# ucas-vg/PointTinyBenchmark

Hardware: AMD Instinct MI355X
Metric: img/s (640x640) CPR R50-FPN fwd+loss (higher is better)
Workload: dtype fp32

## Files before the change

### pointtinybenchmark_amd/csrc/conv_wino.hip

```cpp
#include <type_traits>
#include "common.h"

typedef float f32x2 __attribute__((ext_vector_type(2)));
typedef int i32x4 __attribute__((ext_vector_type(4)));
typedef float f32x2 __attribute__((ext_vector_type(2)));

__device__ __forceinline__ f32x2 pk_add(f32x2 a, f32x2 b) {
    f32x2 r; asm("v_pk_add_f32 %0, %1, %2" : "=v"(r) : "v"(a), "v"(b)); return r;
}
__device__ __forceinline__ f32x2 pk_sub(f32x2 a, f32x2 b) {
    f32x2 r; asm("v_pk_add_f32 %0, %1, %2 neg_lo:[0,1] neg_hi:[0,1]" : "=v"(r) : "v"(a), "v"(b)); return r;
}
__device__ __forceinline__ f32x2 pk_col01(f32x2 t01, f32x2 t23) {
    f32x2 r; asm("v_pk_add_f32 %0, %1, %2 op_sel:[0,0] op_sel_hi:[1,0] neg_lo:[0,1] neg_hi:[0,0]" : "=v"(r) : "v"(t01), "v"(t23)); return r;
}
__device__ __forceinline__ f32x2 pk_col23(f32x2 t01, f32x2 t23) {
    f32x2 r; asm("v_pk_add_f32 %0, %1, %2 op_sel:[1,0] op_sel_hi:[1,1] neg_lo:[1,0] neg_hi:[0,1]" : "=v"(r) : "v"(t01), "v"(t23)); return r;
}
__device__ __forceinline__ f32x2 pk_fma(f32x2 a, f32x2 b, f32x2 c) {
    f32x2 r; asm("v_pk_fma_f32 %0, %1, %2, %3" : "=v"(r) : "v"(a), "v"(b), "v"(c)); return r;
}

struct WinoParams {
    const float* in;
    const float* u;
    float* out;
    const float* scale;
    const float* bias;
    float* gn_part;
    const float* in_a;
    const float* in_b;
    int in_relu, out_b8;
    int N, H, W, Cin, Cout, relu, RY, RX, regions, tilesN, nch;
    int tpx;
};

constexpr int WBUF = 16 * 64 * 8;

__global__ void wino_pack_kernel(const float* __restrict__ w, float* __restrict__ u, int Cin, int Cout, int Kpad) {
    const int idx = blockIdx.x * blockDim.x + threadIdx.x;
    if (idx >= Cin * Cout) return;
    const int ci = idx % Cin, co = idx / Cin;
    float g[3][3];
#pragma unroll
    for (int a = 0; a < 3; ++a)
#pragma unroll
        for (int b = 0; b < 3; ++b) g[a][b] = w[(size_t)co * Kpad + (a * 3 + b) * Cin + ci];
    float t[4][3];
#pragma unroll
    for (int b = 0; b < 3; ++b) {
        t[0][b] = g[0][b];
        t[1][b] = 0.5f * (g[0][b] + g[1][b] + g[2][b]);
        t[2][b] = 0.5f * (g[0][b] - g[1][b] + g[2][b]);
        t[3][b] = g[2][b];
    }
    const int tn = co >> 6, cl = co & 63, chunk = ci >> 3, k = ci & 7, nch = Cin >> 3;
    float* dst = u + ((size_t)(tn * nch + chunk) * 16) * 512 + cl * 8 + 4 * ((k >> 2) ^ ((cl >> 3) & 1)) + (k & 3);
#pragma unroll
    for (int i = 0; i < 4; ++i) {
        dst[(i * 4 + 0) * 512] = t[i][0];
        dst[(i * 4 + 1) * 512] = 0.5f * (t[i][0] + t[i][1] + t[i][2]);
        dst[(i * 4 + 2) * 512] = 0.5f * (t[i][0] - t[i][1] + t[i][2]);
        dst[(i * 4 + 3) * 512] = t[i][2];
    }
}

template <int ABL, bool INB8, bool XF, int TSPREAD = 1, int VAR = 0>
__global__ __launch_bounds__(512, 1) void conv_wino_kernel(WinoParams p) {
    constexpr bool DEEP = (VAR & 1) != 0, UDMA = (VAR & 4) != 0, USINGLE = (VAR & 2) != 0 && !UDMA;
    constexpr int XFMAX = 512;
    constexpr int RAWROW = 148;
    constexpr int RAWBUF = 18 * RAWROW;
    __shared__ __attribute__((aligned(16))) float smem[4 * WBUF + 2 * RAWBUF + (XF ? 4 * XFMAX : 0)];
    float* Vs = smem;
    float* Us = smem + 2 * WBUF;

    const int tid = threadIdx.x, lane = tid & 63;
    const int wave = __builtin_amdgcn_readfirstlane(tid >> 6);
    const int wi = wave & 3;
    const int nh = wave >> 2;

    const int pixbytes = INB8 ? 32 : p.Cin * 4;
    const int chunk_bytes = INB8 ? p.H * p.W * 32 : 32;
    const __amdgpu_buffer_rsrc_t rs_in = __builtin_amdgcn_make_buffer_rsrc(
        const_cast<float*>(p.in), 0, (int)((size_t)p.N * p.H * p.W * p.Cin * 4), 0x00020000);
    const __amdgpu_buffer_rsrc_t rs_u = __builtin_amdgcn_make_buffer_rsrc(
        const_cast<float*>(p.u), 0, (int)((size_t)p.tilesN * p.nch * WBUF * 4), 0x00020000);
    float* Rw = smem + 4 * WBUF;
    float* ABs = smem + 4 * WBUF + 2 * RAWBUF;
    int par = 0;
    int upyx[2], raw_wr[2];
#pragma unroll
    for (int k = 0; k < 2; ++k) {
        const int pix = (tid + 512 * k) >> 1;
        const int py = pix / 18, px = pix - py * 18;
        upyx[k] = py << 8 | px;
        raw_wr[k] = py * RAWROW + px * 8 + (tid & 1) * 4;
    }
    const bool second_unit = wave < 3;
    const bool unit1_live = tid + 512 < 648;
    const int lch = tid & 7, tyl = (tid >> 3) & 7, ltile = wave * 8 + tyl;
    const float* t_rd = Rw + (2 * tyl) * RAWROW + (2 * wave) * 8 + lch;
    const int v_wr = ltile * 8 + 4 * ((lch >> 2) ^ ((ltile >> 3) & 1)) + (lch & 3);
    const int last = p.nch - 1;
    const float relu_floor = (XF && p.in_relu) ? 0.f : -INFINITY;

    struct Tile {
        int rg, tn, n, oy0, ox0, n0;
        int voffA[2];
        unsigned uok;
        bool any_pad, valid;
    };
    const int T = p.regions * p.tilesN;
    const int per = (T + 7) >> 3;
    const int ngrp = p.tpx > 0 ? p.tilesN / p.tpx : 1;
    const int per_r = p.tpx > 0 ? (p.regions * ngrp + 7) / 8 : 0;
    auto setup = [&](int vb) {
        Tile t;
        if (p.tpx > 0) {
            const int x = vb & 7, s = vb >> 3;
            const int sr = s / p.tpx;
            t.rg = (x / ngrp) * per_r + sr;
            t.tn = (x % ngrp) * p.tpx + (s - sr * p.tpx);
            t.valid = sr < per_r && t.rg < p.regions;
            if (!t.valid) { t.rg = 0; t.tn = 0; }
        } else {
            const int tile = (vb & 7) * per + (vb >> 3);
            t.valid = vb < per * 8 && tile < T;
            const int tl = t.valid ? tile : 0;
            t.rg = tl / p.tilesN; t.tn = tl - t.rg * p.tilesN;
        }
        t.n = t.rg / (p.RY * p.RX);
        const int rrem = t.rg - t.n * p.RY * p.RX;
        const int ry = rrem / p.RX, rx = rrem - ry * p.RX;
        t.oy0 = ry * 16; t.ox0 = rx * 16; t.n0 = t.tn * 64;
        const int img_base = INB8 ? (t.n * (p.Cin >> 3)) * p.H * p.W * 32 : t.n * p.H * p.W * p.Cin * 4;
        t.uok = 0;
#pragma unroll
        for (int k = 0; k < 2; ++k) {
            const int iy = t.oy0 - 1 + (upyx[k] >> 8), ix = t.ox0 - 1 + (upyx[k] & 255);
            const bool ok = (k == 0 || unit1_live) & ((unsigned)iy < (unsigned)p.H) & ((unsigned)ix < (unsigned)p.W);
            t.uok |= (ok ? 1u : 0u) << k;
            t.voffA[k] = ok ? img_base + (iy * p.W + ix) * pixbytes + (tid & 1) * 16 : (int)0x80000000;
        }
        t.any_pad = XF && __builtin_amdgcn_ballot_w64(t.uok != (unit1_live ? 3u : 1u)) != 0;
        return t;
    };

    f32x4 sp[2][2];
    f32x4 su[(USINGLE || UDMA) ? 1 : 2][4];
    float tab_a = 0.f, tab_b = 0.f;
    f32x2 d[4][2];
    if (ABL & 9) { sp[0][0] = f32x4{1.f, 1.f, 1.f, 1.f}; sp[0][1] = sp[0][0]; sp[1][0] = sp[0][0]; sp[1][1] = sp[0][0]; }
    Tile cur = setup(blockIdx.x);
    auto ld_a = [&](const Tile& t, int ck, int k) {
        return __builtin_bit_cast(f32x4, __builtin_amdgcn_raw_buffer_load_b128(rs_in, t.voffA[k], ck * chunk_bytes, 0));
    };
    auto ld_u = [&](const Tile& t, int ck, int z) {
        return __builtin_bit_cast(
            f32x4, __builtin_amdgcn_raw_buffer_load_b128(rs_u, tid * 16 + z * 8192, (t.tn * p.nch + ck) * (WBUF * 4), 0));
    };
    auto prefetch = [&](const Tile& t) {
        if (!(ABL & 8)) {
            sp[0][0] = ld_a(t, 0, 0); sp[1][0] = ld_a(t, 1, 0);
            if (second_unit) { sp[0][1] = ld_a(t, 0, 1); sp[1][1] = ld_a(t, 1, 1); }
        }
        if (!UDMA) {
#pragma unroll
            for (int z = 0; z < 4; ++z) { su[0][z] = ld_u(t, 0, z); if (!USINGLE) su[USINGLE ? 0 : 1][z] = ld_u(t, 1, z); }
        }
        if (XF) {
            if (tid < p.Cin) { tab_a = p.in_a[t.n * p.Cin + tid]; tab_b = p.in_b[t.n * p.Cin + tid]; }
        }
    };
    auto g_a = [&](auto set_c, int chunk, int k) {
        constexpr int SET = decltype(set_c)::value;
        if (ABL & 8) return;
        const int ck = chunk < last ? chunk : last;
        if (k == 0 || second_unit) sp[SET][k] = ld_a(cur, ck, k);
    };
    auto g_u = [&](auto set_c, int chunk, int z) {
        constexpr int SET = (USINGLE || UDMA) ? 0 : decltype(set_c)::value;
        if (!UDMA) su[SET][z] = ld_u(cur, chunk < last ? chunk : last, z);
    };
    const int lds_u0 = (int)(unsigned)(size_t)(smem + 2 * WBUF);
    const size_t u_addr = (size_t)p.u;
    const i32x4 rs_u_raw = {(int)(unsigned)u_addr, (int)(unsigned)(u_addr >> 32) & 0xffff,
                            (int)((size_t)p.tilesN * p.nch * WBUF * 4), 0x00020000};
    auto dma_u = [&](int chunk, int buf, int z) {
        const int soff = (cur.tn * p.nch + chunk) * (WBUF * 4);
        const int m0v = lds_u0 + buf * (WBUF * 4) + z * 8192 + wave * 1024;
        asm volatile("s_nop 4\n\ts_mov_b32 m0, %0\n\ts_nop 0\n\tbuffer_load_dwordx4 %1, %2, %3 offen offset:0 lds"
                     :: "s"(m0v), "v"(tid * 16 + z * 8192), "s"(rs_u_raw), "s"(soff) : "memory");
    };
    auto dma_wait = [&](auto npatch_c) {
        constexpr int NP = decltype(npatch_c)::value;
        if (NP == 0) asm volatile("s_waitcnt vmcnt(0)" ::: "memory");
        else if (second_unit) asm volatile("s_waitcnt vmcnt(%0)" :: "n"(2 * NP) : "memory");
        else asm volatile("s_waitcnt vmcnt(%0)" :: "n"(NP) : "memory");
    };
    auto affine = [&](f32x4 v, f32x4 a4, f32x4 b4, int k) {
        if (ABL & 64) v = v * a4 + b4;
        else {
            const f32x2 lo = pk_fma(f32x2{v.x, v.y}, f32x2{a4.x, a4.y}, f32x2{b4.x, b4.y});
            const f32x2 hi = pk_fma(f32x2{v.z, v.w}, f32x2{a4.z, a4.w}, f32x2{b4.z, b4.w});
            v = f32x4{lo.x, lo.y, hi.x, hi.y};
        }
        v.x = fmaxf(v.x, relu_floor); v.y = fmaxf(v.y, relu_floor); v.z = fmaxf(v.z, relu_floor); v.w = fmaxf(v.w, relu_floor);
        if (cur.any_pad) {
            asm volatile("");
            if (!((cur.uok >> k) & 1u)) v = f32x4{0.f, 0.f, 0.f, 0.f};
        }
        return v;
    };
    f32x4 xa4, xb4;
    auto xf_fetch = [&](int chunk) {
        const float* tab = ABs + par * 2 * XFMAX + (chunk < last ? chunk : last) * 8 + (tid & 1) * 4;
        xa4 = *reinterpret_cast<const f32x4*>(tab);
        xb4 = *reinterpret_cast<const f32x4*>(tab + XFMAX);
    };
    auto r_a = [&](auto set_c, int buf, int k) {
        constexpr int SET = decltype(set_c)::value;
        if (k == 1 && !second_unit) return;
        f32x4 v = sp[SET][k];
        if (XF) v = affine(v, xa4, xb4, k);
        if (k == 0 || unit1_live) *reinterpret_cast<f32x4*>(Rw + buf * RAWBUF + raw_wr[k]) = v;
    };
    auto r_a_pro = [&](int chunk01, int k) {
        if (k == 1 && !second_unit) return;
        f32x4 v = chunk01 ? sp[1][k] : sp[0][k];
        if (XF) {
            const float* tab = ABs + par * 2 * XFMAX + chunk01 * 8 + (tid & 1) * 4;
            v = affine(v, *reinterpret_cast<const f32x4*>(tab), *reinterpret_cast<const f32x4*>(tab + XFMAX), k);
        }
        if (k == 0 || unit1_live) *reinterpret_cast<f32x4*>(Rw + chunk01 * RAWBUF + raw_wr[k]) = v;
    };
    auto r_u = [&](auto set_c, int buf, int z) {
        constexpr int SET = (USINGLE || UDMA) ? 0 : decltype(set_c)::value;
        if (!UDMA) *reinterpret_cast<f32x4*>(Us + buf * WBUF + tid * 4 + z * 2048) = su[SET][z];
    };
    auto t_read = [&](int buf, int r) {
#pragma unroll
        for (int s = 0; s < 2; ++s)
            d[r][s] = f32x2{t_rd[buf * RAWBUF + r * RAWROW + (2 * s) * 8], t_rd[buf * RAWBUF + r * RAWROW + (2 * s + 1) * 8]};
    };
    auto t_row = [&](int buf, int i) {
        float* dst = Vs + buf * WBUF + (i * 4) * 512 + v_wr;
        if (ABL & 64) {
            float ts[4];
#pragma unroll
            for (int s = 0; s < 4; ++s) {
                const float d0 = d[0][s >> 1][s & 1], d1 = d[1][s >> 1][s & 1], d2 = d[2][s >> 1][s & 1], d3 = d[3][s >> 1][s & 1];
                ts[s] = i == 0 ? d0 - d2 : i == 1 ? d1 + d2 : i == 2 ? d2 - d1 : d1 - d3;
            }
            dst[0 * 512] = ts[0] - ts[2];
            dst[1 * 512] = ts[1] + ts[2];
            dst[2 * 512] = ts[2] - ts[1];
            dst[3 * 512] = ts[1] - ts[3];
            return;
        }
        f32x2 t[2];
#pragma unroll
        for (int s = 0; s < 2; ++s)
            t[s] = i == 0 ? pk_sub(d[0][s], d[2][s]) : i == 1 ? pk_add(d[1][s], d[2][s]) : i == 2 ? pk_sub(d[2][s], d[1][s])
                                                                                                  : pk_sub(d[1][s], d[3][s]);
        const f32x2 o01 = pk_col01(t[0], t[1]), o23 = pk_col23(t[0], t[1]);
        dst[0 * 512] = o01.x;
        dst[1 * 512] = o01.y;
        dst[2 * 512] = o23.x;
        dst[3 * 512] = o23.y;
    };
    const int l31 = lane & 31, half = lane >> 5;
    const float* a_lds = Vs + (wi * 4 * 64 + l31) * 8 + 4 * (half ^ ((l31 >> 3) & 1));
    const float* b_lds = Us + (wi * 4 * 64 + nh * 32 + l31) * 8 + 4 * (half ^ ((l31 >> 3) & 1));
    using Set0 = std::integral_constant<int, 0>;
    using Set1 = std::integral_constant<int, 1>;

    if (cur.valid) prefetch(cur);
    if (XF) {
        if (tid < p.Cin) { ABs[tid] = tab_a; ABs[XFMAX + tid] = tab_b; }
        __syncthreads();
    }
    for (int vb = blockIdx.x; cur.valid; vb += gridDim.x) {
    const int rg = cur.rg, n = cur.n, oy0 = cur.oy0, ox0 = cur.ox0, n0 = cur.n0;

    f32x16 acc[4][2];
#pragma unroll
    for (int j = 0; j < 4; ++j)
#pragma unroll
        for (int tb = 0; tb < 2; ++tb)
#pragma unroll
            for (int r = 0; r < 16; ++r) acc[j][tb][r] = 0.f;

    f32x4 fa0[2], fb0, fa1[2], fb1;
#define WFRAG(FA, FB, buf, j, z)                                                                                    \
    do {                                                                                                            \
        if ((z) < 2) FA[(z) < 2 ? (z) : 0] = *reinterpret_cast<const f32x4*>(a_lds + (buf) * WBUF + (j) * 512 + ((z) < 2 ? (z) : 0) * 256); \
        else FB = *reinterpret_cast<const f32x4*>(b_lds + (buf) * WBUF + (j) * 512);                                \
    } while (0)
#define WMFMA(FA, FB, j, q) \
    acc[j][(q) & 1] = __builtin_amdgcn_mfma_f32_32x32x2f32(FA[(q) & 1][(q) >> 1], FB[(q) >> 1], acc[j][(q) & 1], 0, 0, 0)
    r_a_pro(0, 0); r_a_pro(0, 1);
    r_a_pro(1, 0); r_a_pro(1, 1);
    if (UDMA) {
#pragma unroll
        for (int z = 0; z < 4; ++z) dma_u(0, 0, z);
#pragma unroll
        for (int z = 0; z < 4; ++z) dma_u(1, 1, z);
    }
#pragma unroll
    for (int z = 0; z < 4; ++z) r_u(Set0{}, 0, z);
    g_a(Set0{}, 2, 0); g_a(Set0{}, 2, 1);
    if (DEEP) { g_a(Set1{}, 3, 0); g_a(Set1{}, 3, 1); }
#pragma unroll
    for (int z = 0; z < 4; ++z) g_u(Set0{}, USINGLE ? 1 : 2, z);
    __syncthreads();
#pragma unroll
    for (int r = 0; r < 4; ++r) t_read(0, r);
#pragma unroll
    for (int i = 0; i < 4; ++i) t_row(0, i);
    if (TSPREAD == 1) {
#pragma unroll
        for (int r = 0; r < 4; ++r) t_read(1, r);
    }
    if (UDMA) dma_wait(std::integral_constant<int, DEEP ? 2 : 1>{});
    __syncthreads();
#pragma unroll
    for (int z = 0; z < 3; ++z) WFRAG(fa0, fb0, 0, 0, z);

    auto iteration = [&](auto nxt_c, int c) {
        const int buf = c & 1;
        const std::integral_constant<int, DEEP ? 1 - decltype(nxt_c)::value : 0> pset_c{};
#pragma unroll
        for (int q = 0; q < 8; ++q) {
            WMFMA(fa0, fb0, 0, q);
            if (q < 3 && !(ABL & 2)) WFRAG(fa1, fb1, buf, 1, q);
            if (!(ABL & 1)) {
                if (TSPREAD == 0 || TSPREAD == 2) { if (q >= 4) t_read(buf ^ 1, q - 4); }
                else { if (q == 3) t_row(buf ^ 1, 0); if (q == 6) t_row(buf ^ 1, 1); }
            }
            __builtin_amdgcn_sched_barrier(0);
        }
#pragma unroll
        for (int q = 0; q < 8; ++q) {
            WMFMA(fa1, fb1, 1, q);
            if (q < 3 && !(ABL & 2)) WFRAG(fa0, fb0, buf, 2, q);
            if (!(ABL & 1)) {
                if (q & 1) r_u(nxt_c, buf ^ 1, q >> 1);
                else if (TSPREAD == 0) t_row(buf ^ 1, q >> 1);
                else if (TSPREAD == 2) {
                    if (q == 0) {
#pragma unroll
                        for (int i = 0; i < 4; ++i) t_row(buf ^ 1, i);
                    }
                }
                else if (q == 2) t_row(buf ^ 1, 2);
                else if (q == 6) t_row(buf ^ 1, 3);
                if (XF && q == 7) xf_fetch(c + 2);
            }
            __builtin_amdgcn_sched_barrier(0);
        }
#pragma unroll
        for (int q = 0; q < 8; ++q) {
            WMFMA(fa0, fb0, 2, q);
            if (q < 3 && !(ABL & 2)) WFRAG(fa1, fb1, buf, 3, q);
            if (!(ABL & 1)) {
                if (q == 3) { r_a(pset_c, buf, 0); if (TSPREAD == 2) r_a(pset_c, buf, 1); }
                if (q == 4 && TSPREAD != 2) r_a(pset_c, buf, 1);
                if (q == 5 || q == 6 || q == 7) g_u(nxt_c, c + (USINGLE ? 2 : 3), q - 5);
            }
            __builtin_amdgcn_sched_barrier(0);
        }
        asm volatile("" ::: "memory");
        if (UDMA) dma_wait(std::integral_constant<int, DEEP ? 1 : 0>{});
        __builtin_amdgcn_s_waitcnt(0xc07f);
        if (!(ABL & 4)) __builtin_amdgcn_s_barrier();
        asm volatile("" ::: "memory");
        __builtin_amdgcn_sched_barrier(0);
#pragma unroll
        for (int q = 0; q < 8; ++q) {
            WMFMA(fa1, fb1, 3, q);
            if (q < 3 && !(ABL & 2)) WFRAG(fa0, fb0, buf ^ 1, 0, q);
            if (!(ABL & 1)) {
                if (UDMA) {
                    if (q < 4 && c + 2 < p.nch) dma_u(c + 2, buf, q);
                    if (q == 4) g_a(pset_c, c + (DEEP ? 4 : 3), 0);
                    if (q == 6) g_a(pset_c, c + (DEEP ? 4 : 3), 1);
                } else {
                    if (q == 3) g_a(pset_c, c + (DEEP ? 4 : 3), 0);
                    if (q == 5) g_a(pset_c, c + (DEEP ? 4 : 3), 1);
                    if (q == 7) g_u(nxt_c, c + (USINGLE ? 2 : 3), 3);
                }
                if (TSPREAD == 1 && q >= 4) t_read(buf, q - 4);
            }
            __builtin_amdgcn_sched_barrier(0);
        }
    };
    for (int c = 0; c < p.nch; c += 2) {
        iteration(Set1{}, c);
        iteration(Set0{}, c + 1);
    }
#undef WFRAG
#undef WMFMA

    if (ABL & 32) {
        asm volatile("" ::"v"(acc[0][0]), "v"(acc[0][1]), "v"(acc[1][0]), "v"(acc[1][1]));
        asm volatile("" ::"v"(acc[2][0]), "v"(acc[2][1]), "v"(acc[3][0]), "v"(acc[3][1]));
        cur = setup(vb + gridDim.x);
        if (cur.valid) prefetch(cur);
        if (XF && tid < p.Cin) { ABs[(par ^ 1) * 2 * XFMAX + tid] = tab_a; ABs[(par ^ 1) * 2 * XFMAX + XFMAX + tid] = tab_b; }
        par ^= 1;
        __syncthreads();
        continue;
    }
    const Tile nxt = setup(vb + gridDim.x);
    if (nxt.valid) prefetch(nxt);
    __syncthreads();
    float* Rs = smem;
#pragma unroll
    for (int tb = 0; tb < 2; ++tb)
#pragma unroll
        for (int r = 0; r < 16; ++r) {
            const int trow = tb * 32 + (r & 3) + 8 * (r >> 2) + 4 * half;
            const float m0 = acc[0][tb][r], m1 = acc[1][tb][r], m2 = acc[2][tb][r], m3 = acc[3][tb][r];
            Rs[((wi * 2 + 0) * 64 + trow) * 64 + nh * 32 + l31] = m0 + m1 + m2;
            Rs[((wi * 2 + 1) * 64 + trow) * 64 + nh * 32 + l31] = m1 - m2 - m3;
        }
    __syncthreads();
    const int c4 = tid & 15;
    const int co = n0 + c4 * 4;
    f32x4 sc = {1.f, 1.f, 1.f, 1.f}, bi = {0.f, 0.f, 0.f, 0.f};
    if (p.scale) sc = *reinterpret_cast<const f32x4*>(p.scale + co);
    if (p.bias) bi = *reinterpret_cast<const f32x4*>(p.bias + co);
    const __amdgpu_buffer_rsrc_t rs_out = __builtin_amdgcn_make_buffer_rsrc(
        p.out, 0, (int)((size_t)p.N * p.H * p.W * p.Cout * 4), 0x00020000);
    f32x4 gs = {0.f, 0.f, 0.f, 0.f}, gq = {0.f, 0.f, 0.f, 0.f};
#pragma unroll
    for (int k = 0; k < 2; ++k) {
        const int t = (tid >> 4) + 32 * k;
        const int oy = oy0 + 2 * (t & 7), ox = ox0 + 2 * (t >> 3);
#pragma unroll
        for (int b = 0; b < 2; ++b) {
            const f32x4 r0 = *reinterpret_cast<const f32x4*>(Rs + ((0 * 2 + b) * 64 + t) * 64 + c4 * 4);
            const f32x4 r1 = *reinterpret_cast<const f32x4*>(Rs + ((1 * 2 + b) * 64 + t) * 64 + c4 * 4);
            const f32x4 r2 = *reinterpret_cast<const f32x4*>(Rs + ((2 * 2 + b) * 64 + t) * 64 + c4 * 4);
            const f32x4 r3 = *reinterpret_cast<const f32x4*>(Rs + ((3 * 2 + b) * 64 + t) * 64 + c4 * 4);
            f32x4 y[2] = {r0 + r1 + r2, r1 - r2 - r3};
#pragma unroll
            for (int a = 0; a < 2; ++a) {
                f32x4 v = y[a] * sc + bi;
                if (p.relu) { v.x = fmaxf(v.x, 0.f); v.y = fmaxf(v.y, 0.f); v.z = fmaxf(v.z, 0.f); v.w = fmaxf(v.w, 0.f); }
                const bool ok = (oy + a < p.H) & (ox + b < p.W);
                const unsigned off = !ok ? 0x80000000u
                    : p.out_b8 ? (unsigned)((((n * (p.Cout >> 3) + (co >> 3)) * p.H + oy + a) * p.W + ox + b) * 8 + (co & 7)) * 4u
                               : (unsigned)(((n * p.H + oy + a) * p.W + ox + b) * p.Cout + co) * 4u;
                if (!(ABL & 16)) __builtin_amdgcn_raw_buffer_store_b128(__builtin_bit_cast(__attribute__((ext_vector_type(4))) unsigned, v), rs_out, (int)off, 0, 0);
                if (p.gn_part && ok) { gs += v; gq += v * v; }
            }
        }
    }
    if (p.gn_part) {
#pragma unroll
        for (int e = 0; e < 4; ++e) {
            gs[e] += __shfl_xor(gs[e], 16, 64); gs[e] += __shfl_xor(gs[e], 32, 64);
            gq[e] += __shfl_xor(gq[e], 16, 64); gq[e] += __shfl_xor(gq[e], 32, 64);
        }
        __syncthreads();
        if (lane < 16) {
#pragma unroll
            for (int e = 0; e < 4; ++e) {
                smem[(wave * 64 + c4 * 4 + e) * 2 + 0] = gs[e];
                smem[(wave * 64 + c4 * 4 + e) * 2 + 1] = gq[e];
            }
        }
        __syncthreads();
        if (tid < 64) {
            float s = 0.f, q = 0.f;
#pragma unroll
            for (int w8 = 0; w8 < 8; ++w8) { s += smem[(w8 * 64 + tid) * 2]; q += smem[(w8 * 64 + tid) * 2 + 1]; }
            float* dst = p.gn_part + ((size_t)rg * p.Cout + n0 + tid) * 2;
            dst[0] = s; dst[1] = q;
        }
    }
    if (XF && tid < p.Cin) {
        ABs[(par ^ 1) * 2 * XFMAX + tid] = tab_a;
        ABs[(par ^ 1) * 2 * XFMAX + XFMAX + tid] = tab_b;
    }
    par ^= 1;
    __syncthreads();
    cur = nxt;
    }
}

#ifdef CPR_BENCH_HOOKS
static int wino_sched = 0, wino_ablate = 0, wino_var = -1, wino_tpx = -1;
extern "C" int cpr_wino_set_variant(int sched, int ablate) {
    CPR_CHECK_ARG(sched >= 0 && sched <= 2 && ablate >= 0 && ablate <= 64);
    wino_sched = sched;
    wino_ablate = ablate;
    return CPR_OK;
}
extern "C" int cpr_wino_set_staging(int var, int tpx) {
    CPR_CHECK_ARG(var >= -1 && var <= 5 && tpx >= -1 && tpx <= 2);
    wino_var = var;
    wino_tpx = tpx;
    return CPR_OK;
}
#else
constexpr int wino_sched = 0, wino_ablate = 0, wino_var = -1, wino_tpx = -1;
#endif
constexpr int WINO_VAR_DEFAULT = 4, WINO_TPX_DEFAULT = 0;
extern "C" int cpr_wino_pack_weights(const float* wgt, float* u, int Cin, int Cout, int Kpad, hipStream_t stream) {
    CPR_CHECK_ARG(wgt && u && Cin > 0 && Cout > 0 && Cin % 8 == 0 && Cout % 64 == 0 && Kpad >= 9 * Cin);
    hipLaunchKernelGGL(wino_pack_kernel, dim3(cdiv(Cin * Cout, 256)), dim3(256), 0, stream, wgt, u, Cin, Cout, Kpad);
    CPR_LAUNCH_STATUS();
}
static int wino_fwd_launch(const float* in, const float* u, float* out, const float* scale, const float* bias,
                           const float* in_a, const float* in_b, float* gn_part, int N, int H, int W, int Cin,
                           int Cout, int flags, int in_relu, int layout, hipStream_t stream) {
    CPR_CHECK_ARG(in && u && out && N > 0 && H > 0 && W > 0);
    CPR_CHECK_ARG(Cin > 0 && Cout > 0 && Cin % 16 == 0 && Cout % 64 == 0 && Cin >= 32);
    CPR_CHECK_ARG((flags & ~CPR_CONV_RELU) == 0 && (layout & ~3) == 0);
    if (in_a) CPR_CHECK_ARG(in_b && Cin <= 512);
    if ((long long)N * H * W * Cin * 4 >= (1ll << 31) || (long long)N * H * W * Cout * 4 >= (1ll << 31)) return CPR_ERR_UNSUPPORTED;
    WinoParams p;
    p.in = in; p.u = u; p.out = out; p.scale = scale; p.bias = bias; p.gn_part = gn_part;
    p.in_a = in_a; p.in_b = in_b; p.in_relu = in_relu; p.out_b8 = (layout & CPR_WINO_OUT_B8) ? 1 : 0;
    p.N = N; p.H = H; p.W = W; p.Cin = Cin; p.Cout = Cout; p.relu = flags & CPR_CONV_RELU;
    p.RY = (H + 15) / 16; p.RX = (W + 15) / 16;
    p.regions = N * p.RY * p.RX; p.tilesN = Cout / 64; p.nch = Cin / 8;
    const long long T = (long long)p.regions * p.tilesN;
    if (T >= (1ll << 30)) return CPR_ERR_UNSUPPORTED;
    static int cu_of_device[64] = {};
    int dev = 0, ncu = 256;
    if (hipGetDevice(&dev) == hipSuccess && dev >= 0 && dev < 64) {
        if (cu_of_device[dev] == 0) {
            int v = 0;
            if (hipDeviceGetAttribute(&v, hipDeviceAttributeMultiprocessorCount, dev) == hipSuccess && v > 0) cu_of_device[dev] = v;
        }
        if (cu_of_device[dev] > 0) ncu = cu_of_device[dev];
    }
    ncu = (ncu + 7) / 8 * 8;
    int grid = (int)((T + 7) / 8 * 8);
    if (grid > ncu) grid = ncu;
    const bool b8 = (layout & CPR_WINO_IN_B8) != 0, xf = in_a != nullptr;
    p.tpx = wino_tpx >= 0 ? wino_tpx : WINO_TPX_DEFAULT;
    if (p.tpx > 0 && !(p.tilesN % p.tpx == 0 && 8 % (p.tilesN / p.tpx) == 0)) p.tpx = 0;
    if (p.tpx > 0) {
        const long long per_r = ((long long)p.regions * (p.tilesN / p.tpx) + 7) / 8;
        const long long vbs = 8 * per_r * p.tpx;
        if (vbs < grid) grid = (int)vbs;
    }
    const int var = wino_var >= 0 ? wino_var : WINO_VAR_DEFAULT;
#define WLAUNCHV(A_, F_, V_)                                                                                                      \
    do {                                                                                                                         \
        constexpr int TX_ = F_ == 2 ? 2 : 0 ^ F_, TP_ = F_ == 2 ? 2 : 1 ^ F_;                                                     \
        if (b8 && xf) hipLaunchKernelGGL((conv_wino_kernel<A_, true, true, TX_, V_>), dim3(grid), dim3(512), 0, stream, p);       \
        else if (b8) hipLaunchKernelGGL((conv_wino_kernel<A_, true, false, TP_, V_>), dim3(grid), dim3(512), 0, stream, p);       \
        else if (xf) hipLaunchKernelGGL((conv_wino_kernel<A_, false, true, TX_, V_>), dim3(grid), dim3(512), 0, stream, p);       \
        else hipLaunchKernelGGL((conv_wino_kernel<A_, false, false, TP_, V_>), dim3(grid), dim3(512), 0, stream, p);              \
    } while (0)
#define WLAUNCH(A_, F_) WLAUNCHV(A_, F_, WINO_VAR_DEFAULT)
#ifdef CPR_BENCH_HOOKS
    if ((var != WINO_VAR_DEFAULT || wino_sched == 2) && !wino_ablate) {
        switch (var * 3 + wino_sched) {
            case 0: WLAUNCHV(0, 0, 0); break;
            case 1: WLAUNCHV(0, 1, 0); break;
            case 2: WLAUNCHV(0, 2, 0); break;
            case 6: WLAUNCHV(0, 0, 2); break;
            case 7: WLAUNCHV(0, 1, 2); break;
            case 8: WLAUNCHV(0, 2, 2); break;
            case 9: WLAUNCHV(0, 0, 3); break;
            case 10: WLAUNCHV(0, 1, 3); break;
            case 11: WLAUNCHV(0, 2, 3); break;
            case 12: WLAUNCHV(0, 0, 4); break;
            case 13: WLAUNCHV(0, 1, 4); break;
            case 14: WLAUNCHV(0, 2, 4); break;
            default: return CPR_ERR_UNSUPPORTED;
        }
    } else if (wino_ablate || wino_sched) {
        switch (wino_ablate) {
            case 0: WLAUNCH(0, 1); break;
            case 1: WLAUNCH(1, 0); break;
            case 2: WLAUNCH(2, 0); break;
            case 4: WLAUNCH(4, 0); break;
            case 8: WLAUNCH(8, 0); break;
            case 16: WLAUNCH(16, 0); break;
            case 32: WLAUNCH(32, 0); break;
            case 64: WLAUNCH(64, 0); break;
            default: WLAUNCH(7, 0); break;
        }
    } else
#endif
    WLAUNCH(0, 0);
#undef WLAUNCH
#undef WLAUNCHV
    CPR_LAUNCH_STATUS();
}

extern "C" int cpr_conv3x3_wino_fwd(const float* in, const float* u, float* out, const float* scale, const float* bias,
                                    const float* in_a, const float* in_b, float* gn_part, int N, int H, int W, int Cin,
                                    int Cout, int flags, int in_relu, int layout, hipStream_t stream) {
    CPR_CHECK_ARG(N > 0 && H > 0 && W > 0 && Cin > 0 && Cout > 0);
    const int per = cpr_images_per_launch(N, (long long)H * W * cpr_max2(Cin, Cout) * 4);
    if (per <= 0) return CPR_ERR_UNSUPPORTED;
    const size_t slots = (size_t)((H + 15) / 16) * ((W + 15) / 16);
    for (int n0 = 0; n0 < N; n0 += per) {
        const int n = N - n0 < per ? N - n0 : per;
        const int rc = wino_fwd_launch(in + (size_t)n0 * H * W * Cin, u, out + (size_t)n0 * H * W * Cout, scale, bias,
                                       in_a ? in_a + (size_t)n0 * Cin : nullptr, in_b ? in_b + (size_t)n0 * Cin : nullptr,
                                       gn_part ? gn_part + (size_t)n0 * slots * Cout * 2 : nullptr, n, H, W, Cin, Cout, flags,
                                       in_relu, layout, stream);
        if (rc != CPR_OK) return rc;
    }
    return CPR_OK;
}
```

Baseline: 898.7.

## Overlap Winograd output epilogue with next tile's prologue staging

```diff
diff --git a/pointtinybenchmark_amd/csrc/conv_wino.hip b/pointtinybenchmark_amd/csrc/conv_wino.hip
--- a/pointtinybenchmark_amd/csrc/conv_wino.hip
+++ b/pointtinybenchmark_amd/csrc/conv_wino.hip
@@ -68,6 +68,7 @@
 template <int ABL, bool INB8, bool XF, int TSPREAD = 1, int VAR = 0>
 __global__ __launch_bounds__(512, 1) void conv_wino_kernel(WinoParams p) {
     constexpr bool DEEP = (VAR & 1) != 0, UDMA = (VAR & 4) != 0, USINGLE = (VAR & 2) != 0 && !UDMA;
+    constexpr bool OVERLAP = XF;
     constexpr int XFMAX = 512;
     constexpr int RAWROW = 148;
     constexpr int RAWBUF = 18 * RAWROW;
@@ -160,16 +161,18 @@
         return __builtin_bit_cast(
             f32x4, __builtin_amdgcn_raw_buffer_load_b128(rs_u, tid * 16 + z * 8192, (t.tn * p.nch + ck) * (WBUF * 4), 0));
     };
-    auto prefetch = [&](const Tile& t) {
+    auto prefetch = [&](const Tile& t, bool table) {
         if (!(ABL & 8)) {
-            sp[0][0] = ld_a(t, 0, 0); sp[1][0] = ld_a(t, 1, 0);
-            if (second_unit) { sp[0][1] = ld_a(t, 0, 1); sp[1][1] = ld_a(t, 1, 1); }
+            sp[0][0] = ld_a(t, 0, 0);
+            if (second_unit) sp[0][1] = ld_a(t, 0, 1);
+            sp[1][0] = ld_a(t, 1, 0);
+            if (second_unit) sp[1][1] = ld_a(t, 1, 1);
         }
         if (!UDMA) {
 #pragma unroll
             for (int z = 0; z < 4; ++z) { su[0][z] = ld_u(t, 0, z); if (!USINGLE) su[USINGLE ? 0 : 1][z] = ld_u(t, 1, z); }
         }
-        if (XF) {
+        if (XF && table) {
             if (tid < p.Cin) { tab_a = p.in_a[t.n * p.Cin + tid]; tab_b = p.in_b[t.n * p.Cin + tid]; }
         }
     };
@@ -199,6 +202,12 @@
         else if (second_unit) asm volatile("s_waitcnt vmcnt(%0)" :: "n"(2 * NP) : "memory");
         else asm volatile("s_waitcnt vmcnt(%0)" :: "n"(NP) : "memory");
     };
+    auto dma_wait_boundary = [&](auto npatch_c) {
+        constexpr int NP = (ABL & 8) ? 0 : decltype(npatch_c)::value;
+        constexpr int OLD = ((ABL & 16) ? 0 : 8) + 4;
+        if (second_unit) asm volatile("s_waitcnt vmcnt(%0)" :: "n"(OLD + 2 * NP) : "memory");
+        else asm volatile("s_waitcnt vmcnt(%0)" :: "n"(OLD + NP) : "memory");
+    };
     auto affine = [&](f32x4 v, f32x4 a4, f32x4 b4, int k) {
         if (ABL & 64) v = v * a4 + b4;
         else {
@@ -276,13 +285,48 @@
     using Set0 = std::integral_constant<int, 0>;
     using Set1 = std::integral_constant<int, 1>;
 
-    if (cur.valid) prefetch(cur);
+    auto head_plain = [&]() {
+        r_a_pro(0, 0); r_a_pro(0, 1);
+        r_a_pro(1, 0); r_a_pro(1, 1);
+        if (UDMA) {
+#pragma unroll
+            for (int z = 0; z < 4; ++z) dma_u(0, 0, z);
+#pragma unroll
+            for (int z = 0; z < 4; ++z) dma_u(1, 1, z);
+        }
+#pragma unroll
+        for (int z = 0; z < 4; ++z) r_u(Set0{}, 0, z);
+        g_a(Set0{}, 2, 0); g_a(Set0{}, 2, 1);
+        if (DEEP) { g_a(Set1{}, 3, 0); g_a(Set1{}, 3, 1); }
+#pragma unroll
+        for (int z = 0; z < 4; ++z) g_u(Set0{}, USINGLE ? 1 : 2, z);
+        __syncthreads();
+#pragma unroll
+        for (int r = 0; r < 4; ++r) t_read(0, r);
+#pragma unroll
+        for (int i = 0; i < 4; ++i) t_row(0, i);
+        if (TSPREAD == 1) {
+#pragma unroll
+            for (int r = 0; r < 4; ++r) t_read(1, r);
+        }
+        if (UDMA) dma_wait(std::integral_constant<int, (ABL & 8) ? 0 : DEEP ? 2 : 1>{});
+        __syncthreads();
+    };
+
+    if (cur.valid) prefetch(cur, true);
     if (XF) {
         if (tid < p.Cin) { ABs[tid] = tab_a; ABs[XFMAX + tid] = tab_b; }
         __syncthreads();
     }
+    if (cur.valid) head_plain();
     for (int vb = blockIdx.x; cur.valid; vb += gridDim.x) {
     const int rg = cur.rg, n = cur.n, oy0 = cur.oy0, ox0 = cur.ox0, n0 = cur.n0;
+
+    const int c4 = tid & 15;
+    const int co = n0 + c4 * 4;
+    f32x4 sc = {1.f, 1.f, 1.f, 1.f}, bi = {0.f, 0.f, 0.f, 0.f};
+    if (p.scale) sc = *reinterpret_cast<const f32x4*>(p.scale + co);
+    if (p.bias) bi = *reinterpret_cast<const f32x4*>(p.bias + co);
 
     f32x16 acc[4][2];
 #pragma unroll
@@ -300,31 +344,6 @@
     } while (0)
 #define WMFMA(FA, FB, j, q) \
     acc[j][(q) & 1] = __builtin_amdgcn_mfma_f32_32x32x2f32(FA[(q) & 1][(q) >> 1], FB[(q) >> 1], acc[j][(q) & 1], 0, 0, 0)
-    r_a_pro(0, 0); r_a_pro(0, 1);
-    r_a_pro(1, 0); r_a_pro(1, 1);
-    if (UDMA) {
-#pragma unroll
-        for (int z = 0; z < 4; ++z) dma_u(0, 0, z);
-#pragma unroll
-        for (int z = 0; z < 4; ++z) dma_u(1, 1, z);
-    }
-#pragma unroll
-    for (int z = 0; z < 4; ++z) r_u(Set0{}, 0, z);
-    g_a(Set0{}, 2, 0); g_a(Set0{}, 2, 1);
-    if (DEEP) { g_a(Set1{}, 3, 0); g_a(Set1{}, 3, 1); }
-#pragma unroll
-    for (int z = 0; z < 4; ++z) g_u(Set0{}, USINGLE ? 1 : 2, z);
-    __syncthreads();
-#pragma unroll
-    for (int r = 0; r < 4; ++r) t_read(0, r);
-#pragma unroll
-    for (int i = 0; i < 4; ++i) t_row(0, i);
-    if (TSPREAD == 1) {
-#pragma unroll
-        for (int r = 0; r < 4; ++r) t_read(1, r);
-    }
-    if (UDMA) dma_wait(std::integral_constant<int, DEEP ? 2 : 1>{});
-    __syncthreads();
 #pragma unroll
     for (int z = 0; z < 3; ++z) WFRAG(fa0, fb0, 0, 0, z);
 
@@ -396,10 +415,12 @@
             __builtin_amdgcn_sched_barrier(0);
         }
     };
-    for (int c = 0; c < p.nch; c += 2) {
+    int c = 0;
+    do {
         iteration(Set1{}, c);
         iteration(Set0{}, c + 1);
-    }
+        c += 2;
+    } while (c < p.nch);
 #undef WFRAG
 #undef WMFMA
 
@@ -407,44 +428,114 @@
         asm volatile("" ::"v"(acc[0][0]), "v"(acc[0][1]), "v"(acc[1][0]), "v"(acc[1][1]));
         asm volatile("" ::"v"(acc[2][0]), "v"(acc[2][1]), "v"(acc[3][0]), "v"(acc[3][1]));
         cur = setup(vb + gridDim.x);
-        if (cur.valid) prefetch(cur);
+        if (cur.valid) prefetch(cur, true);
         if (XF && tid < p.Cin) { ABs[(par ^ 1) * 2 * XFMAX + tid] = tab_a; ABs[(par ^ 1) * 2 * XFMAX + XFMAX + tid] = tab_b; }
         par ^= 1;
         __syncthreads();
+        if (cur.valid) head_plain();
         continue;
     }
-    const Tile nxt = setup(vb + gridDim.x);
-    if (nxt.valid) prefetch(nxt);
-    __syncthreads();
-    float* Rs = smem;
-#pragma unroll
-    for (int tb = 0; tb < 2; ++tb)
-#pragma unroll
-        for (int r = 0; r < 16; ++r) {
-            const int trow = tb * 32 + (r & 3) + 8 * (r >> 2) + 4 * half;
-            const float m0 = acc[0][tb][r], m1 = acc[1][tb][r], m2 = acc[2][tb][r], m3 = acc[3][tb][r];
-            Rs[((wi * 2 + 0) * 64 + trow) * 64 + nh * 32 + l31] = m0 + m1 + m2;
-            Rs[((wi * 2 + 1) * 64 + trow) * 64 + nh * 32 + l31] = m1 - m2 - m3;
-        }
-    __syncthreads();
-    const int c4 = tid & 15;
-    const int co = n0 + c4 * 4;
-    f32x4 sc = {1.f, 1.f, 1.f, 1.f}, bi = {0.f, 0.f, 0.f, 0.f};
-    if (p.scale) sc = *reinterpret_cast<const f32x4*>(p.scale + co);
-    if (p.bias) bi = *reinterpret_cast<const f32x4*>(p.bias + co);
     const __amdgpu_buffer_rsrc_t rs_out = __builtin_amdgcn_make_buffer_rsrc(
         p.out, 0, (int)((size_t)p.N * p.H * p.W * p.Cout * 4), 0x00020000);
-    f32x4 gs = {0.f, 0.f, 0.f, 0.f}, gq = {0.f, 0.f, 0.f, 0.f};
-#pragma unroll
-    for (int k = 0; k < 2; ++k) {
-        const int t = (tid >> 4) + 32 * k;
-        const int oy = oy0 + 2 * (t & 7), ox = ox0 + 2 * (t >> 3);
-#pragma unroll
-        for (int b = 0; b < 2; ++b) {
-            const f32x4 r0 = *reinterpret_cast<const f32x4*>(Rs + ((0 * 2 + b) * 64 + t) * 64 + c4 * 4);
-            const f32x4 r1 = *reinterpret_cast<const f32x4*>(Rs + ((1 * 2 + b) * 64 + t) * 64 + c4 * 4);
-            const f32x4 r2 = *reinterpret_cast<const f32x4*>(Rs + ((2 * 2 + b) * 64 + t) * 64 + c4 * 4);
-            const f32x4 r3 = *reinterpret_cast<const f32x4*>(Rs + ((3 * 2 + b) * 64 + t) * 64 + c4 * 4);
+    if (!OVERLAP) {
+        cur = setup(vb + gridDim.x);
+        if (cur.valid) prefetch(cur, true);
+        __syncthreads();
+        float* Rs = smem;
+#pragma unroll
+        for (int tb = 0; tb < 2; ++tb)
+#pragma unroll
+            for (int r = 0; r < 16; ++r) {
+                const int trow = tb * 32 + (r & 3) + 8 * (r >> 2) + 4 * half;
+                const float m0 = acc[0][tb][r], m1 = acc[1][tb][r], m2 = acc[2][tb][r], m3 = acc[3][tb][r];
+                Rs[((wi * 2 + 0) * 64 + trow) * 64 + nh * 32 + l31] = m0 + m1 + m2;
+                Rs[((wi * 2 + 1) * 64 + trow) * 64 + nh * 32 + l31] = m1 - m2 - m3;
+            }
+        __syncthreads();
+        f32x4 gs = {0.f, 0.f, 0.f, 0.f}, gq = {0.f, 0.f, 0.f, 0.f};
+#pragma unroll
+        for (int k = 0; k < 2; ++k) {
+            const int t = (tid >> 4) + 32 * k;
+            const int oy = oy0 + 2 * (t & 7), ox = ox0 + 2 * (t >> 3);
+#pragma unroll
+            for (int b = 0; b < 2; ++b) {
+                const f32x4 r0 = *reinterpret_cast<const f32x4*>(Rs + ((0 * 2 + b) * 64 + t) * 64 + c4 * 4);
+                const f32x4 r1 = *reinterpret_cast<const f32x4*>(Rs + ((1 * 2 + b) * 64 + t) * 64 + c4 * 4);
+                const f32x4 r2 = *reinterpret_cast<const f32x4*>(Rs + ((2 * 2 + b) * 64 + t) * 64 + c4 * 4);
+                const f32x4 r3 = *reinterpret_cast<const f32x4*>(Rs + ((3 * 2 + b) * 64 + t) * 64 + c4 * 4);
+                f32x4 y[2] = {r0 + r1 + r2, r1 - r2 - r3};
+#pragma unroll
+                for (int a = 0; a < 2; ++a) {
+                    f32x4 v = y[a] * sc + bi;
+                    if (p.relu) { v.x = fmaxf(v.x, 0.f); v.y = fmaxf(v.y, 0.f); v.z = fmaxf(v.z, 0.f); v.w = fmaxf(v.w, 0.f); }
+                    const bool ok = (oy + a < p.H) & (ox + b < p.W);
+                    const unsigned off = !ok ? 0x80000000u
+                        : p.out_b8 ? (unsigned)((((n * (p.Cout >> 3) + (co >> 3)) * p.H + oy + a) * p.W + ox + b) * 8 + (co & 7)) * 4u
+                                   : (unsigned)(((n * p.H + oy + a) * p.W + ox + b) * p.Cout + co) * 4u;
+                    if (!(ABL & 16)) __builtin_amdgcn_raw_buffer_store_b128(__builtin_bit_cast(__attribute__((ext_vector_type(4))) unsigned, v), rs_out, (int)off, 0, 0);
+                    if (p.gn_part && ok) { gs += v; gq += v * v; }
+                }
+            }
+        }
+        if (p.gn_part) {
+#pragma unroll
+            for (int e = 0; e < 4; ++e) {
+                gs[e] += __shfl_xor(gs[e], 16, 64); gs[e] += __shfl_xor(gs[e], 32, 64);
+                gq[e] += __shfl_xor(gq[e], 16, 64); gq[e] += __shfl_xor(gq[e], 32, 64);
+            }
+            __syncthreads();
+            if (lane < 16) {
+#pragma unroll
+                for (int e = 0; e < 4; ++e) {
+                    smem[(wave * 64 + c4 * 4 + e) * 2 + 0] = gs[e];
+                    smem[(wave * 64 + c4 * 4 + e) * 2 + 1] = gq[e];
+                }
+            }
+            __syncthreads();
+            if (tid < 64) {
+                float s = 0.f, q = 0.f;
+#pragma unroll
+                for (int w8 = 0; w8 < 8; ++w8) { s += smem[(w8 * 64 + tid) * 2]; q += smem[(w8 * 64 + tid) * 2 + 1]; }
+                float* dst = p.gn_part + ((size_t)rg * p.Cout + n0 + tid) * 2;
+                dst[0] = s; dst[1] = q;
+            }
+        }
+        __syncthreads();
+        if (cur.valid) head_plain();
+        continue;
+    }
+    cur = setup(vb + gridDim.x);
+    const bool stage = cur.valid;
+    const bool new_table = XF && stage && cur.n != n;
+    if (stage) {
+        if (UDMA) {
+#pragma unroll
+            for (int z = 0; z < 4; ++z) dma_u(0, 0, z);
+        }
+        prefetch(cur, new_table);
+    }
+    float* r_wr = smem + WBUF + (wi >> 1) * 2 * WBUF + (wi & 1) * 4096 + nh * 32 + l31;
+    auto r_pass = [&](int b) {
+#pragma unroll
+        for (int tb = 0; tb < 2; ++tb)
+#pragma unroll
+            for (int r = 0; r < 16; ++r) {
+                const int trow = tb * 32 + (r & 3) + 8 * (r >> 2) + 4 * half;
+                const float m0 = acc[0][tb][r], m1 = acc[1][tb][r], m2 = acc[2][tb][r], m3 = acc[3][tb][r];
+                r_wr[trow * 64] = b == 0 ? m0 + m1 + m2 : m1 - m2 - m3;
+            }
+    };
+    f32x4 yv[2][2][2];
+    auto y_pass = [&](int b) {
+#pragma unroll
+        for (int k = 0; k < 2; ++k) {
+            const int t = (tid >> 4) + 32 * k;
+            const int oy = oy0 + 2 * (t & 7), ox = ox0 + 2 * (t >> 3);
+            const float* r_rd = smem + WBUF + t * 64 + c4 * 4;
+            const f32x4 r0 = *reinterpret_cast<const f32x4*>(r_rd);
+            const f32x4 r1 = *reinterpret_cast<const f32x4*>(r_rd + 4096);
+            const f32x4 r2 = *reinterpret_cast<const f32x4*>(r_rd + 2 * WBUF);
+            const f32x4 r3 = *reinterpret_cast<const f32x4*>(r_rd + 2 * WBUF + 4096);
             f32x4 y[2] = {r0 + r1 + r2, r1 - r2 - r3};
 #pragma unroll
             for (int a = 0; a < 2; ++a) {
@@ -455,40 +546,87 @@
                     : p.out_b8 ? (unsigned)((((n * (p.Cout >> 3) + (co >> 3)) * p.H + oy + a) * p.W + ox + b) * 8 + (co & 7)) * 4u
                                : (unsigned)(((n * p.H + oy + a) * p.W + ox + b) * p.Cout + co) * 4u;
                 if (!(ABL & 16)) __builtin_amdgcn_raw_buffer_store_b128(__builtin_bit_cast(__attribute__((ext_vector_type(4))) unsigned, v), rs_out, (int)off, 0, 0);
-                if (p.gn_part && ok) { gs += v; gq += v * v; }
-            }
-        }
-    }
+                yv[b][k][a] = v;
+            }
+        }
+    };
+
+    r_pass(0);
+    if (new_table) {
+        if (tid < p.Cin) { ABs[(par ^ 1) * 2 * XFMAX + tid] = tab_a; ABs[(par ^ 1) * 2 * XFMAX + XFMAX + tid] = tab_b; }
+        par ^= 1;
+    }
+    __syncthreads();
+    y_pass(0);
+    __syncthreads();
+    r_pass(1);
+    if (stage) {
+        r_a_pro(0, 0); r_a_pro(0, 1);
+        r_a_pro(1, 0); r_a_pro(1, 1);
+#pragma unroll
+        for (int z = 0; z < 4; ++z) r_u(Set0{}, 0, z);
+    }
+    __syncthreads();
+    if (stage) {
+#pragma unroll
+        for (int r = 0; r < 4; ++r) t_read(0, r);
+#pragma unroll
+        for (int i = 0; i < 4; ++i) t_row(0, i);
+    }
+    y_pass(1);
+    float* Gs = ABs + (par ^ 1) * 2 * XFMAX;
     if (p.gn_part) {
+        f32x4 gs = {0.f, 0.f, 0.f, 0.f}, gq = {0.f, 0.f, 0.f, 0.f};
+#pragma unroll
+        for (int k = 0; k < 2; ++k) {
+            const int t = (tid >> 4) + 32 * k;
+            const int oy = oy0 + 2 * (t & 7), ox = ox0 + 2 * (t >> 3);
+#pragma unroll
+            for (int b = 0; b < 2; ++b)
+#pragma unroll
+                for (int a = 0; a < 2; ++a) {
+                    const f32x4 v = yv[b][k][a];
+                    const bool ok = (oy + a < p.H) & (ox + b < p.W);
+                    if (ok) { gs += v; gq += v * v; }
+                }
+        }
 #pragma unroll
         for (int e = 0; e < 4; ++e) {
             gs[e] += __shfl_xor(gs[e], 16, 64); gs[e] += __shfl_xor(gs[e], 32, 64);
             gq[e] += __shfl_xor(gq[e], 16, 64); gq[e] += __shfl_xor(gq[e], 32, 64);
         }
+        if (lane < 16) {
+#pragma unroll
+            for (int e = 0; e < 4; ++e) {
+                Gs[(wave * 64 + c4 * 4 + e) * 2 + 0] = gs[e];
+                Gs[(wave * 64 + c4 * 4 + e) * 2 + 1] = gq[e];
+            }
+        }
+    }
+    __syncthreads();
+    if (p.gn_part && tid < 64) {
+        float s = 0.f, q = 0.f;
+#pragma unroll
+        for (int w8 = 0; w8 < 8; ++w8) { s += Gs[(w8 * 64 + tid) * 2]; q += Gs[(w8 * 64 + tid) * 2 + 1]; }
+        float* dst = p.gn_part + ((size_t)rg * p.Cout + n0 + tid) * 2;
+        dst[0] = s; dst[1] = q;
+    }
+    if (stage) {
+        if (UDMA) {
+#pragma unroll
+            for (int z = 0; z < 4; ++z) dma_u(1, 1, z);
+        }
+        g_a(Set0{}, 2, 0); g_a(Set0{}, 2, 1);
+        if (DEEP) { g_a(Set1{}, 3, 0); g_a(Set1{}, 3, 1); }
+#pragma unroll
+        for (int z = 0; z < 4; ++z) g_u(Set0{}, USINGLE ? 1 : 2, z);
+        if (TSPREAD == 1) {
+#pragma unroll
+            for (int r = 0; r < 4; ++r) t_read(1, r);
+        }
+        if (UDMA) dma_wait_boundary(std::integral_constant<int, DEEP ? 2 : 1>{});
         __syncthreads();
-        if (lane < 16) {
-#pragma unroll
-            for (int e = 0; e < 4; ++e) {
-                smem[(wave * 64 + c4 * 4 + e) * 2 + 0] = gs[e];
-                smem[(wave * 64 + c4 * 4 + e) * 2 + 1] = gq[e];
-            }
-        }
-        __syncthreads();
-        if (tid < 64) {
-            float s = 0.f, q = 0.f;
-#pragma unroll
-            for (int w8 = 0; w8 < 8; ++w8) { s += smem[(w8 * 64 + tid) * 2]; q += smem[(w8 * 64 + tid) * 2 + 1]; }
-            float* dst = p.gn_part + ((size_t)rg * p.Cout + n0 + tid) * 2;
-            dst[0] = s; dst[1] = q;
-        }
-    }
-    if (XF && tid < p.Cin) {
-        ABs[(par ^ 1) * 2 * XFMAX + tid] = tab_a;
-        ABs[(par ^ 1) * 2 * XFMAX + XFMAX + tid] = tab_b;
-    }
-    par ^= 1;
-    __syncthreads();
-    cur = nxt;
+    }
     }
 }
 
```

Result: no change. 899.7 (median of 2 runs) (+0.1%).
